# BatsResearch/menghini-neurips23-code

Measured on AMD Instinct MI355X. Metric: images/sec CLIP ViT-B/16 encode+prompt-step, higher is better.
Workload: dtype f16

## Files before the change

menghini-neurips23-code_amd/csrc/attention_split.hip:

```cpp
#include <math.h>

#include "common.h"

__device__ __forceinline__ int vt_index_fwd_s(int key, int d) { return vt_index(key, ((d >> 2) & 3) * 16 + (d >> 4) * 4 + (d & 3)); }

__device__ __forceinline__ void split8(const f32x4 a, const f32x4 b, half8& hi, half8& lo) {
    half4 h0, l0, h1, l1;
    split_f16x4(a, h0, l0);
    split_f16x4(b, h1, l1);
    hi = (half8){h0[0], h0[1], h0[2], h0[3], h1[0], h1[1], h1[2], h1[3]};
    lo = (half8){l0[0], l0[1], l0[2], l0[3], l1[0], l1[1], l1[2], l1[3]};
}

template <int KVC, bool CAUSAL, int NW>
__global__ __launch_bounds__(NW * 64) void attn_fwd_split_kernel(const float* __restrict__ qkv, half_t* __restrict__ out, int S, int H) {
    constexpr int SP = KVC * 32;
    constexpr float LOG2E = 1.4426950408889634f;
    constexpr float INV = 1.0f / (float)GRIP_SPLIT_LO_SCALE;
    extern __shared__ __attribute__((aligned(16))) char smem[];
    half_t* Kh = (half_t*)smem;
    half_t* Kl = Kh + SP * 64;
    half_t* Vh = Kl + SP * 64;
    half_t* Vl = Vh + SP * 64;

    const int tid = threadIdx.x, lane = tid & 63, wave = tid >> 6;
    const int D = H * 64;
    const int b = blockIdx.x / H, h = blockIdx.x - b * H;
    const size_t ld = (size_t)3 * D;
    const float* base = qkv + (size_t)b * S * ld + h * 64;
    const int li = lane & 15, lg = lane >> 4;
    const int n_qt = (S + 15) >> 4;

    for (int idx = tid; idx < SP * 8; idx += NW * 64) {
        const int row = idx >> 3, chunk = idx & 7;
        f32x4 a = {0.f, 0.f, 0.f, 0.f}, c = {0.f, 0.f, 0.f, 0.f};
        if (row < S) {
            const f32x4* p = (const f32x4*)(base + (size_t)row * ld + D + chunk * 8);
            a = p[0];
            c = p[1];
        }
        half8 hi, lo;
        split8(a, c, hi, lo);
        const int o = row * 64 + ((chunk ^ (row & 7)) * 8);
        *(half8*)(Kh + o) = hi;
        *(half8*)(Kl + o) = lo;
    }
    for (int idx = tid; idx < ((SP / 2 + 31) / 32) * 256; idx += NW * 64) {
        const int lane_rp = idx & 31, chunk = ((idx >> 5) & 1) + 2 * ((idx >> 6) & 3), rblk = idx >> 8;
        const int r0 = 2 * (rblk * 32 + lane_rp);
        if (r0 >= SP) continue;
        f32x4 z = {0.f, 0.f, 0.f, 0.f};
        f32x4 a0 = z, a1 = z, b0 = z, b1 = z;
        if (r0 < S) { const f32x4* p = (const f32x4*)(base + (size_t)r0 * ld + 2 * D + chunk * 8); a0 = p[0]; a1 = p[1]; }
        if (r0 + 1 < S) { const f32x4* p = (const f32x4*)(base + (size_t)(r0 + 1) * ld + 2 * D + chunk * 8); b0 = p[0]; b1 = p[1]; }
        half8 h0, l0, h1, l1;
        split8(a0, a1, h0, l0);
        split8(b0, b1, h1, l1);
#pragma unroll
        for (int j = 0; j < 8; ++j) {
            const int o = vt_index_fwd_s(r0, chunk * 8 + j);
            *(half2v*)(Vh + o) = (half2v){h0[j], h1[j]};
            *(half2v*)(Vl + o) = (half2v){l0[j], l1[j]};
        }
    }
    __syncthreads();

    for (int qt = wave; qt < n_qt; qt += NW) {
        asm volatile("" ::: "memory");
        const int qrow = qt * 16 + li;
        const int qr = qrow < S ? qrow : S - 1;
        half8 qh[2], ql[2];
#pragma unroll
        for (int kk = 0; kk < 2; ++kk) {
            const f32x4* p = (const f32x4*)(base + (size_t)qr * ld + (kk * 4 + lg) * 8);
            split8(p[0] * 0.125f, p[1] * 0.125f, qh[kk], ql[kk]);
        }
        f32x4 sc[2 * KVC];
        float m = -INFINITY;
#pragma unroll
        for (int t = 0; t < 2 * KVC; ++t) {
            f32x4 acc = {0.f, 0.f, 0.f, 0.f}, cor = {0.f, 0.f, 0.f, 0.f};
#pragma unroll
            for (int kk = 0; kk < 2; ++kk) {
                const int o = (t * 16 + li) * 64 + (((kk * 4 + lg) ^ (lane & 7)) * 8);
                const half8 kh = *(const half8*)(Kh + o), kl = *(const half8*)(Kl + o);
                acc = __builtin_amdgcn_mfma_f32_16x16x32_f16(kh, qh[kk], acc, 0, 0, 0);
                cor = __builtin_amdgcn_mfma_f32_16x16x32_f16(kl, qh[kk], cor, 0, 0, 0);
                cor = __builtin_amdgcn_mfma_f32_16x16x32_f16(kh, ql[kk], cor, 0, 0, 0);
            }
            acc += cor * INV;
            if (CAUSAL || t >= 2 * (KVC - 1)) {
#pragma unroll
                for (int r = 0; r < 4; ++r) {
                    const int kv = t * 16 + lg * 4 + r;
                    if (kv >= S || (CAUSAL && kv > qrow)) acc[r] = -INFINITY;
                }
            }
            m = fmaxf(fmaxf(fmaxf(m, acc[0]), fmaxf(acc[1], acc[2])), acc[3]);
            sc[t] = acc;
        }
        m = fmaxf(m, __shfl_xor(m, 16));
        m = fmaxf(m, __shfl_xor(m, 32));
        const float m2 = m * LOG2E;
#pragma unroll
        for (int t = 0; t < 2 * KVC; ++t)
#pragma unroll
            for (int r = 0; r < 4; ++r) sc[t][r] = __builtin_amdgcn_exp2f(__builtin_fmaf(sc[t][r], LOG2E, -m2));

        const half8 ones = {1, 1, 1, 1, 1, 1, 1, 1};
        f32x4 sum_h = {0.f, 0.f, 0.f, 0.f}, sum_l = {0.f, 0.f, 0.f, 0.f};
        f32x4 o[4], oc[4];
#pragma unroll
        for (int nf = 0; nf < 4; ++nf) { o[nf] = (f32x4){0.f, 0.f, 0.f, 0.f}; oc[nf] = (f32x4){0.f, 0.f, 0.f, 0.f}; }
#pragma unroll
        for (int c = 0; c < KVC; ++c) {
            half8 ph, pl;
            split8(sc[2 * c], sc[2 * c + 1], ph, pl);
#pragma unroll
            for (int nf = 0; nf < 4; ++nf) {
                const int vo = (c * 4 + nf) * 512 + (lg * 16 + (li ^ lg)) * 8;
                const half8 vh = *(const half8*)(Vh + vo), vl = *(const half8*)(Vl + vo);
                o[nf] = __builtin_amdgcn_mfma_f32_16x16x32_f16(vh, ph, o[nf], 0, 0, 0);
                oc[nf] = __builtin_amdgcn_mfma_f32_16x16x32_f16(vl, ph, oc[nf], 0, 0, 0);
                oc[nf] = __builtin_amdgcn_mfma_f32_16x16x32_f16(vh, pl, oc[nf], 0, 0, 0);
            }
            sum_h = __builtin_amdgcn_mfma_f32_16x16x32_f16(ones, ph, sum_h, 0, 0, 0);
            sum_l = __builtin_amdgcn_mfma_f32_16x16x32_f16(ones, pl, sum_l, 0, 0, 0);
        }
        if (qrow < S) {
            const float inv = 1.0f / (sum_h[0] + sum_l[0] * INV);
            half_t* orow = out + (size_t)((size_t)b * S + qrow) * 2 * D;
            const int col = h * 64 + lg * 16;
            half_t* op = orow + (col >> 5) * 64 + (col & 31);
            half8 hi0, lo0, hi1, lo1;
            split8((o[0] + oc[0] * INV) * inv, (o[1] + oc[1] * INV) * inv, hi0, lo0);
            split8((o[2] + oc[2] * INV) * inv, (o[3] + oc[3] * INV) * inv, hi1, lo1);
            *(half8*)op = hi0;
            *(half8*)(op + 8) = hi1;
            *(half8*)(op + 32) = lo0;
            *(half8*)(op + 40) = lo1;
        }
    }
}

bool attention_split_supported(int S) { return S >= 1 && S <= 320; }

int launch_attention_fwd_split(const float* qkv, void* out, int B, int S, int H, int causal, hipStream_t s) {
    GRIP_REQUIRE(attention_split_supported(S) && B >= 1 && H >= 1, "attention_split: bad shape B=%d S=%d H=%d (S <= 320)", B, S, H);
    const int kvc = (S + 31) / 32;
    const size_t lds = (size_t)4 * kvc * 32 * 64 * sizeof(half_t);
#define GRIP_ATT_CASE(K)                                                                                                                     \
    case K: {                                                                                                                                \
        static bool configured = false;                                                                                                      \
        if (!configured) {                                                                                                                   \
            GRIP_CHECK_HIP(hipFuncSetAttribute((const void*)attn_fwd_split_kernel<K, false, (K >= 4 ? 8 : 4)>, hipFuncAttributeMaxDynamicSharedMemorySize, (int)lds)); \
            GRIP_CHECK_HIP(hipFuncSetAttribute((const void*)attn_fwd_split_kernel<K, true, (K >= 4 ? 8 : 4)>, hipFuncAttributeMaxDynamicSharedMemorySize, (int)lds));  \
            configured = true;                                                                                                               \
        }                                                                                                                                    \
        if (causal) hipLaunchKernelGGL((attn_fwd_split_kernel<K, true, (K >= 4 ? 8 : 4)>), dim3(B * H), dim3((K >= 4 ? 8 : 4) * 64), lds, s, qkv, (half_t*)out, S, H); \
        else hipLaunchKernelGGL((attn_fwd_split_kernel<K, false, (K >= 4 ? 8 : 4)>), dim3(B * H), dim3((K >= 4 ? 8 : 4) * 64), lds, s, qkv, (half_t*)out, S, H);       \
    } break;
    switch (kvc) {
        GRIP_ATT_CASE(1) GRIP_ATT_CASE(2) GRIP_ATT_CASE(3) GRIP_ATT_CASE(4) GRIP_ATT_CASE(5)
        GRIP_ATT_CASE(6) GRIP_ATT_CASE(7) GRIP_ATT_CASE(8) GRIP_ATT_CASE(9) GRIP_ATT_CASE(10)
        default: GRIP_REQUIRE(false, "attention_split: S = %d out of range", S);
    }
#undef GRIP_ATT_CASE
    GRIP_CHECK_HIP(hipGetLastError());
    return GRIP_OK;
}
```

Measured before the change: 20820.

## Software-pipeline LDS reads, Q prefetch and softmax in split attention kernel

Restructures the split-precision attention kernel so that global K/V loads are all issued before any conversion or LDS stores. Q for the next tile is prefetched into registers, and K/V fragments are double-buffered from LDS one step ahead of the MFMAs. The exponentials and hi/lo splitting of the next chunk are interleaved with the PV MFMAs using sched_group_barrier hints. A fully masked final key tile is skipped. This hides LDS and global latency and overlaps VALU with matrix ops, at the cost of higher register pressure and heavy reliance on compiler scheduling hints.

```diff
diff --git a/menghini-neurips23-code_amd/csrc/attention_split.hip b/menghini-neurips23-code_amd/csrc/attention_split.hip
--- a/menghini-neurips23-code_amd/csrc/attention_split.hip
+++ b/menghini-neurips23-code_amd/csrc/attention_split.hip
@@ -31,63 +31,108 @@
     const int li = lane & 15, lg = lane >> 4;
     const int n_qt = (S + 15) >> 4;
 
-    for (int idx = tid; idx < SP * 8; idx += NW * 64) {
-        const int row = idx >> 3, chunk = idx & 7;
-        f32x4 a = {0.f, 0.f, 0.f, 0.f}, c = {0.f, 0.f, 0.f, 0.f};
+    const f32x4 zero4 = {0.f, 0.f, 0.f, 0.f};
+
+    f32x4 q_next[4];
+    auto load_q = [&](int qt) {
+        const int qrow = qt * 16 + li;
+        const int qr = qrow < S ? qrow : S - 1;
+#pragma unroll
+        for (int kk = 0; kk < 2; ++kk) {
+            const f32x4* p = (const f32x4*)(base + (size_t)qr * ld + (kk * 4 + lg) * 8);
+            q_next[2 * kk] = p[0];
+            q_next[2 * kk + 1] = p[1];
+        }
+    };
+    load_q(wave < n_qt ? wave : 0);
+
+    constexpr int NT = NW * 64;
+    constexpr int K_N = SP * 8, K_IT = (K_N + NT - 1) / NT;
+    constexpr int V_N = ((SP / 2 + 31) / 32) * 256, V_IT = (V_N + NT - 1) / NT;
+    f32x4 kf[K_IT][2], vf[V_IT][4];
+#pragma unroll
+    for (int i = 0; i < K_IT; ++i) {
+        const int idx = tid + i * NT, row = idx >> 3, chunk = idx & 7;
+        kf[i][0] = zero4;
+        kf[i][1] = zero4;
         if (row < S) {
             const f32x4* p = (const f32x4*)(base + (size_t)row * ld + D + chunk * 8);
-            a = p[0];
-            c = p[1];
-        }
-        half8 hi, lo;
-        split8(a, c, hi, lo);
-        const int o = row * 64 + ((chunk ^ (row & 7)) * 8);
-        *(half8*)(Kh + o) = hi;
-        *(half8*)(Kl + o) = lo;
-    }
-    for (int idx = tid; idx < ((SP / 2 + 31) / 32) * 256; idx += NW * 64) {
+            kf[i][0] = p[0];
+            kf[i][1] = p[1];
+        }
+    }
+#pragma unroll
+    for (int i = 0; i < V_IT; ++i) {
+        const int idx = tid + i * NT;
         const int lane_rp = idx & 31, chunk = ((idx >> 5) & 1) + 2 * ((idx >> 6) & 3), rblk = idx >> 8;
         const int r0 = 2 * (rblk * 32 + lane_rp);
-        if (r0 >= SP) continue;
-        f32x4 z = {0.f, 0.f, 0.f, 0.f};
-        f32x4 a0 = z, a1 = z, b0 = z, b1 = z;
-        if (r0 < S) { const f32x4* p = (const f32x4*)(base + (size_t)r0 * ld + 2 * D + chunk * 8); a0 = p[0]; a1 = p[1]; }
-        if (r0 + 1 < S) { const f32x4* p = (const f32x4*)(base + (size_t)(r0 + 1) * ld + 2 * D + chunk * 8); b0 = p[0]; b1 = p[1]; }
-        half8 h0, l0, h1, l1;
-        split8(a0, a1, h0, l0);
-        split8(b0, b1, h1, l1);
-#pragma unroll
-        for (int j = 0; j < 8; ++j) {
-            const int o = vt_index_fwd_s(r0, chunk * 8 + j);
-            *(half2v*)(Vh + o) = (half2v){h0[j], h1[j]};
-            *(half2v*)(Vl + o) = (half2v){l0[j], l1[j]};
+        vf[i][0] = zero4; vf[i][1] = zero4; vf[i][2] = zero4; vf[i][3] = zero4;
+        if (r0 < S) { const f32x4* p = (const f32x4*)(base + (size_t)r0 * ld + 2 * D + chunk * 8); vf[i][0] = p[0]; vf[i][1] = p[1]; }
+        if (r0 + 1 < S) { const f32x4* p = (const f32x4*)(base + (size_t)(r0 + 1) * ld + 2 * D + chunk * 8); vf[i][2] = p[0]; vf[i][3] = p[1]; }
+    }
+#pragma unroll
+    for (int i = 0; i < K_IT; ++i) {
+        const int idx = tid + i * NT, row = idx >> 3, chunk = idx & 7;
+        if (idx < K_N) {
+            half8 hi, lo;
+            split8(kf[i][0], kf[i][1], hi, lo);
+            const int o = row * 64 + ((chunk ^ (row & 7)) * 8);
+            *(half8*)(Kh + o) = hi;
+            *(half8*)(Kl + o) = lo;
+        }
+    }
+#pragma unroll
+    for (int i = 0; i < V_IT; ++i) {
+        const int idx = tid + i * NT;
+        const int lane_rp = idx & 31, chunk = ((idx >> 5) & 1) + 2 * ((idx >> 6) & 3), rblk = idx >> 8;
+        const int r0 = 2 * (rblk * 32 + lane_rp);
+        if (idx < V_N && r0 < SP) {
+            half8 h0, l0, h1, l1;
+            split8(vf[i][0], vf[i][1], h0, l0);
+            split8(vf[i][2], vf[i][3], h1, l1);
+#pragma unroll
+            for (int j = 0; j < 8; ++j) {
+                const int o = vt_index_fwd_s(r0, chunk * 8 + j);
+                *(half2v*)(Vh + o) = (half2v){h0[j], h1[j]};
+                *(half2v*)(Vl + o) = (half2v){l0[j], l1[j]};
+            }
         }
     }
     __syncthreads();
+
+    half8 kh[2][2], kl[2][2], vh[2], vl[2];
+    int ko_h[2], ko_l[2];
+#pragma unroll
+    for (int kk = 0; kk < 2; ++kk) {
+        ko_h[kk] = li * 64 + (((kk * 4 + lg) ^ (lane & 7)) * 8);
+        ko_l[kk] = ko_h[kk] + SP * 64;
+    }
+    int vo_h = 2 * SP * 64 + (lg * 16 + (li ^ lg)) * 8, vo_l = vo_h + SP * 64;
+    asm volatile("" : "+v"(ko_h[0]), "+v"(ko_h[1]), "+v"(ko_l[0]), "+v"(ko_l[1]), "+v"(vo_h), "+v"(vo_l));
+    auto read_k = [&](int t) {
+#pragma unroll
+        for (int kk = 0; kk < 2; ++kk) {
+            kh[t & 1][kk] = *(const half8*)(Kh + ko_h[kk] + t * 1024);
+            kl[t & 1][kk] = *(const half8*)(Kh + ko_l[kk] + t * 1024);
+        }
+    };
+    auto read_v = [&](int j) {
+        vh[j & 1] = *(const half8*)(Kh + vo_h + j * 512);
+        vl[j & 1] = *(const half8*)(Kh + vo_l + j * 512);
+    };
+    const bool last_dead = S <= (2 * KVC - 1) * 16;
 
     for (int qt = wave; qt < n_qt; qt += NW) {
         asm volatile("" ::: "memory");
         const int qrow = qt * 16 + li;
-        const int qr = qrow < S ? qrow : S - 1;
+        read_k(0);
         half8 qh[2], ql[2];
 #pragma unroll
-        for (int kk = 0; kk < 2; ++kk) {
-            const f32x4* p = (const f32x4*)(base + (size_t)qr * ld + (kk * 4 + lg) * 8);
-            split8(p[0] * 0.125f, p[1] * 0.125f, qh[kk], ql[kk]);
-        }
+        for (int kk = 0; kk < 2; ++kk) split8(q_next[2 * kk] * 0.125f, q_next[2 * kk + 1] * 0.125f, qh[kk], ql[kk]);
+        if (qt + NW < n_qt) load_q(qt + NW);
         f32x4 sc[2 * KVC];
         float m = -INFINITY;
-#pragma unroll
-        for (int t = 0; t < 2 * KVC; ++t) {
-            f32x4 acc = {0.f, 0.f, 0.f, 0.f}, cor = {0.f, 0.f, 0.f, 0.f};
-#pragma unroll
-            for (int kk = 0; kk < 2; ++kk) {
-                const int o = (t * 16 + li) * 64 + (((kk * 4 + lg) ^ (lane & 7)) * 8);
-                const half8 kh = *(const half8*)(Kh + o), kl = *(const half8*)(Kl + o);
-                acc = __builtin_amdgcn_mfma_f32_16x16x32_f16(kh, qh[kk], acc, 0, 0, 0);
-                cor = __builtin_amdgcn_mfma_f32_16x16x32_f16(kl, qh[kk], cor, 0, 0, 0);
-                cor = __builtin_amdgcn_mfma_f32_16x16x32_f16(kh, ql[kk], cor, 0, 0, 0);
-            }
+        auto finish = [&](int t, f32x4 acc, const f32x4 cor) {
             acc += cor * INV;
             if (CAUSAL || t >= 2 * (KVC - 1)) {
 #pragma unroll
@@ -97,32 +142,74 @@
                 }
             }
             m = fmaxf(fmaxf(fmaxf(m, acc[0]), fmaxf(acc[1], acc[2])), acc[3]);
+            asm volatile("" : "+v"(m));
             sc[t] = acc;
-        }
+        };
+        f32x4 pacc = zero4, pcor = zero4;
+#pragma unroll
+        for (int t = 0; t < 2 * KVC; ++t) {
+            __builtin_amdgcn_sched_barrier(0);
+            if (t + 1 < 2 * KVC) read_k(t + 1);
+            f32x4 acc = {0.f, 0.f, 0.f, 0.f}, cor = {0.f, 0.f, 0.f, 0.f};
+            if (!(t == 2 * KVC - 1 && last_dead)) {
+#pragma unroll
+                for (int kk = 0; kk < 2; ++kk) {
+                    acc = __builtin_amdgcn_mfma_f32_16x16x32_f16(kh[t & 1][kk], qh[kk], acc, 0, 0, 0);
+                    cor = __builtin_amdgcn_mfma_f32_16x16x32_f16(kl[t & 1][kk], qh[kk], cor, 0, 0, 0);
+                    cor = __builtin_amdgcn_mfma_f32_16x16x32_f16(kh[t & 1][kk], ql[kk], cor, 0, 0, 0);
+                }
+            }
+            if (t > 0) finish(t - 1, pacc, pcor);
+            pacc = acc;
+            pcor = cor;
+            __builtin_amdgcn_sched_group_barrier(0x100, 4, 0);
+#pragma unroll
+            for (int i = 0; i < 6; ++i) {
+                __builtin_amdgcn_sched_group_barrier(0x008, 1, 0);
+                __builtin_amdgcn_sched_group_barrier(0x402, 3, 0);
+            }
+        }
+        __builtin_amdgcn_sched_barrier(0);
+        if (last_dead) sc[2 * KVC - 1] = (f32x4){-INFINITY, -INFINITY, -INFINITY, -INFINITY};
+        else finish(2 * KVC - 1, pacc, pcor);
         m = fmaxf(m, __shfl_xor(m, 16));
         m = fmaxf(m, __shfl_xor(m, 32));
         const float m2 = m * LOG2E;
-#pragma unroll
-        for (int t = 0; t < 2 * KVC; ++t)
+        read_v(0);
+        auto exps = [&](int t) {
+            if (t == 2 * KVC - 1 && last_dead) { sc[t] = zero4; return; }
 #pragma unroll
             for (int r = 0; r < 4; ++r) sc[t][r] = __builtin_amdgcn_exp2f(__builtin_fmaf(sc[t][r], LOG2E, -m2));
+        };
+        exps(0);
+        exps(1);
 
         const half8 ones = {1, 1, 1, 1, 1, 1, 1, 1};
         f32x4 sum_h = {0.f, 0.f, 0.f, 0.f}, sum_l = {0.f, 0.f, 0.f, 0.f};
         f32x4 o[4], oc[4];
 #pragma unroll
         for (int nf = 0; nf < 4; ++nf) { o[nf] = (f32x4){0.f, 0.f, 0.f, 0.f}; oc[nf] = (f32x4){0.f, 0.f, 0.f, 0.f}; }
+        half8 ph_n, pl_n;
+        split8(sc[0], sc[1], ph_n, pl_n);
 #pragma unroll
         for (int c = 0; c < KVC; ++c) {
-            half8 ph, pl;
-            split8(sc[2 * c], sc[2 * c + 1], ph, pl);
+            const half8 ph = ph_n, pl = pl_n;
 #pragma unroll
             for (int nf = 0; nf < 4; ++nf) {
-                const int vo = (c * 4 + nf) * 512 + (lg * 16 + (li ^ lg)) * 8;
-                const half8 vh = *(const half8*)(Vh + vo), vl = *(const half8*)(Vl + vo);
-                o[nf] = __builtin_amdgcn_mfma_f32_16x16x32_f16(vh, ph, o[nf], 0, 0, 0);
-                oc[nf] = __builtin_amdgcn_mfma_f32_16x16x32_f16(vl, ph, oc[nf], 0, 0, 0);
-                oc[nf] = __builtin_amdgcn_mfma_f32_16x16x32_f16(vh, pl, oc[nf], 0, 0, 0);
+                const int j = c * 4 + nf;
+                __builtin_amdgcn_sched_barrier(0);
+                if (j + 1 < 4 * KVC) read_v(j + 1);
+                o[nf] = __builtin_amdgcn_mfma_f32_16x16x32_f16(vh[j & 1], ph, o[nf], 0, 0, 0);
+                oc[nf] = __builtin_amdgcn_mfma_f32_16x16x32_f16(vl[j & 1], ph, oc[nf], 0, 0, 0);
+                oc[nf] = __builtin_amdgcn_mfma_f32_16x16x32_f16(vh[j & 1], pl, oc[nf], 0, 0, 0);
+                if (c + 1 < KVC && nf < 2) exps(2 * c + 2 + nf);
+                if (c + 1 < KVC && nf == 2) split8(sc[2 * c + 2], sc[2 * c + 3], ph_n, pl_n);
+                __builtin_amdgcn_sched_group_barrier(0x100, 2, 0);
+#pragma unroll
+                for (int i = 0; i < 3; ++i) {
+                    __builtin_amdgcn_sched_group_barrier(0x008, 1, 0);
+                    __builtin_amdgcn_sched_group_barrier(0x402, 6, 0);
+                }
             }
             sum_h = __builtin_amdgcn_mfma_f32_16x16x32_f16(ones, ph, sum_h, 0, 0, 0);
             sum_l = __builtin_amdgcn_mfma_f32_16x16x32_f16(ones, pl, sum_l, 0, 0, 0);
```

Measured after the change: 20880, median of 6. About the same (+0.3%).
